# ictnlp/StreamSpeech

Measured on AMD Instinct MI355X. Metric: real-time factor (RTFx = audio seconds / wall seconds) + utterances/sec, offline S2ST fr-en, higher is better.
Workload: dtype f32

## Files before the change

streamspeech_amd/csrc/conv_c64w.hip:

```cpp
#include "slab_common.hpp"

#include <type_traits>

namespace ss {

using u32x4 = __attribute__((ext_vector_type(4))) unsigned;

#ifndef CW_TIMING
#define CW_TIMING 0
#endif
#if CW_TIMING
__device__ unsigned long long g_cw_dbg[1024 * 8];
#define CW_STAMP(k) do { if (t == 0) { const unsigned long long _n = __builtin_amdgcn_s_memtime(); cw_acc[k] += _n - cw_last; cw_last = _n; } } while (0)
#else
#define CW_STAMP(k) do { } while (0)
#endif

namespace {
constexpr int CW_MAXSEG = 256;
constexpr int CW_MAXROWS = 320;
constexpr int CW_MAXROWS_128 = 192;
[[maybe_unused]] constexpr int CW_NUM_RECORDS = 0x7ffffff0;
constexpr int cw_bme(int dil, int rows = 256) { return rows == 128 ? (dil == 1 ? 128 : dil == 3 ? 126 : 120) : (dil == 1 ? 256 : dil == 3 ? 252 : 240); }
[[maybe_unused]] __host__ __device__ constexpr int cw_nc(int kind) { return kind == 0 ? 4 : kind == 1 ? 2 : 3; }
[[maybe_unused]] __host__ __device__ constexpr int cw_slot(int kind, int n) { return kind == 0 ? n : kind == 1 ? (n == 0 ? 0 : 3) : (n == 2 ? 3 : n); }
[[maybe_unused]] __host__ __device__ constexpr int cw_ja(int kind, int n) { return kind == 0 ? (n == 3 ? 1 : n) : kind == 1 ? n : (n == 0 ? 0 : 1); }
[[maybe_unused]] __host__ __device__ constexpr int cw_jb(int kind, int n) { return kind == 0 ? (n == 2 ? 1 : n == 3 ? 3 : 2) : kind == 1 ? n : (n == 2 ? 2 : 1); }
[[maybe_unused]] __host__ __device__ constexpr int cw_op(int kind, int n) { return kind == 0 ? (n == 1 ? 1 : -1) : kind == 1 ? 0 : (n == 1 ? 0 : -1); }
}

__global__ void wino_pack_kernel(const float* __restrict__ W, float* __restrict__ WW, int C, int taps, int groups) {
  const int n = C * groups * C;
  for (int idx = blockIdx.x * blockDim.x + threadIdx.x; idx < n; idx += gridDim.x * blockDim.x) {
    const int ci = idx % C, g = (idx / C) % groups, co = idx / (C * groups);
    const float* w = W + (size_t)co * taps * C + ci;
    const float w0 = 3 * g < taps ? w[(size_t)(3 * g) * C] : 0.f;
    const float w1 = 3 * g + 1 < taps ? w[(size_t)(3 * g + 1) * C] : 0.f;
    const float w2 = 3 * g + 2 < taps ? w[(size_t)(3 * g + 2) * C] : 0.f;
    float* o = WW + (size_t)co * groups * 4 * C + (size_t)g * 4 * C + ci;
    const int left = taps - 3 * g;
    if (left >= 3) {
      o[0] = w0;
      o[C] = 0.5f * ((w0 + w1) + w2);
      o[2 * C] = 0.5f * ((w0 - w1) + w2);
      o[3 * C] = w2;
    } else if (left == 2) {
      o[0] = w0; o[C] = w0 + w1; o[2 * C] = 0.f; o[3 * C] = w1;
    } else {
      o[0] = w0; o[C] = 0.f; o[2 * C] = 0.f; o[3 * C] = -w0;
    }
  }
}

template <int DIL, int CH, int TAIL, int ROWS = 256>
__global__ __launch_bounds__(CH >= 128 ? 512 : 256, CH >= 128 ? 1 : CH == 64 ? 2 : 3) void conv_c64w_kernel(const GemmArgs p, const int groups, const int slab_rows) {
#if __HIP_DEVICE_COMPILE__
  constexpr int CS = CH == 256 ? 128 : CH;
  constexpr int KH = CH / CS;
  constexpr int C = CH, LDA = CS + 4, CT = CH >= 64 ? 4 : CH / 16, CB = CS / 16, RING = 2 * CT, TPR = CS / 4;
  constexpr int NT = CH >= 128 ? 512 : 256, RPP = NT / TPR;
  static_assert(ROWS == 256 || (ROWS == 128 && CH == 256), "half-height blocks: the 256-channel form only");
// ... 332 lines not shown
```

streamspeech_amd/csrc/debug_ops.hip:

```cpp
#include "model_internal.hpp"
#include "ctc_align.hpp"
#include "ctc_beam.hpp"

static int op_bind_wino(GemmArgs& a, void* stream) {
  static thread_local std::map<hipStream_t, DevBuf> wino_tmps;
  DevBuf& wino_tmp = wino_tmps[(hipStream_t)stream];
  const int N = a.N, Cin = a.Cin, taps = a.taps;
  if ((conv_c64w_enabled() && N == 64 && Cin == 64 && taps >= 3 && conv_c64_eligible(a)) ||
      (conv_c128w_enabled() && N == 128 && Cin == 128 && taps >= 3 && a.same_rows && !a.glu) ||
      (conv_c256w_enabled() && N == 256 && Cin == 256 && taps >= 3 && a.same_rows && !a.glu) ||
      (conv_c32w_enabled() && N == 32 && Cin == 32 && taps >= 3 && conv_c32_eligible(a))) {
    RET(wino_tmp.ensure((size_t)N * ((taps + 2) / 3) * 4 * N * sizeof(float)));
    RET(launch_wino_pack(a.W, wino_tmp.f(), N, taps, (hipStream_t)stream));
    a.Wwino = wino_tmp.f();
  }
  return SS_OK;
}

extern "C" int ss_op_conv_gemm(void* stream, const float* dA, int lda, const float* dW, const float* dbias,
                               const float* dR, int ldr, const float* dR2, int ldr2, float* dC, int ldc, int M,
                               int N, int Cin, int taps, int dil, int stride, int pad, int in_len, int chunk,
                               int in_act, float in_slope, int act, float alpha, float div, int glu) {
  GemmArgs a;
  a.A = dA; a.lda = lda; a.W = dW; a.bias = dbias; a.R = dR; a.ldr = ldr; a.R2 = dR2; a.ldr2 = ldr2; a.C = dC; a.ldc = ldc;
  a.M = M; a.N = N; a.Cin = Cin; a.taps = taps; a.dil = dil; a.stride = stride; a.pad = pad; a.in_len = in_len;
  a.chunk = chunk; a.in_act = in_act; a.in_slope = in_slope; a.act = act; a.alpha = alpha; a.div = div; a.glu = glu;
  a.same_rows = (stride == 1 && M == in_len) ? 1 : 0;
  RET(op_bind_wino(a, stream));
  return launch_conv_gemm(a, (hipStream_t)stream);
}

static void op_fill_conv(GemmArgs& a, const ss_op_conv_args* x) {
  a.A = x->A; a.W = x->W; a.bias = x->bias; a.R = x->R; a.R2 = x->R2; a.C = x->C; a.C2 = x->C2;
  a.lda = x->lda; a.ldc = x->ldc; a.ldr = x->ldr; a.ldr2 = x->ldr2; a.ldc2 = x->ldc2;
  a.M = x->M; a.N = x->N; a.Cin = x->Cin; a.taps = x->taps; a.dil = x->dil; a.stride = x->stride; a.pad = x->pad;
  a.in_len = x->in_len; a.chunk = x->chunk;
  a.in_act = x->in_act; a.in_slope = x->in_slope; a.act = x->act; a.act_slope = x->act_slope; a.alpha = x->alpha; a.div = x->div;
  a.c2_slope = x->c2_slope; a.glu = x->glu;
  a.segs = x->segs; a.nseg = x->nseg; a.max_seg_out = x->max_seg_out; a.same_rows = x->same_rows;
}
extern "C" int ss_op_conv_gemm_ex(void* stream, const ss_op_conv_args* x) {
  if (!x) return SS_ERR_ARG;
  GemmArgs a;
  op_fill_conv(a, x);
// ... 71 lines not shown
}
extern "C" int ss_op_ln_linear(void* stream, const float* dX, int ldx, const float* ln_g, const float* ln_b, const float* dW,
                               const float* dbias, const float* dR, int ldr, float* dC, int ldc, int M, int N, int K, int act,
                               float alpha, int glu) {
  GemmArgs a;
  a.A = dX; a.lda = ldx; a.W = dW; a.bias = dbias; a.R = dR; a.ldr = ldr; a.C = dC; a.ldc = ldc;
  a.M = M; a.N = N; a.Cin = K; a.in_len = M; a.act = act; a.alpha = alpha; a.glu = glu; a.same_rows = 1;
  a.ln_g = ln_g; a.ln_b = ln_b;
  return launch_conv_gemm(a, (hipStream_t)stream);
}
extern "C" int ss_op_ln_linear_ex(void* stream, const float* dX, int ldx, const float* ln_g, const float* ln_b, float* ln_out,
                                  const float* dW, const float* dbias, const float* dR, int ldr, float* dC, int ldc, int M, int N, int K,
                                  int act, float alpha, int glu, int canon) {
  if (canon < 0 || canon > 2 || (ln_g == nullptr) != (ln_b == nullptr) || (ln_out && !ln_g)) return SS_ERR_ARG;
  GemmArgs a;
  a.A = dX; a.lda = ldx; a.W = dW; a.bias = dbias; a.R = dR; a.ldr = ldr; a.C = dC; a.ldc = ldc;
  a.M = M; a.N = N; a.Cin = K; a.in_len = M; a.act = act; a.alpha = alpha; a.glu = glu; a.same_rows = 1;
  a.ln_g = ln_g; a.ln_b = ln_b; a.ln_out = ln_out; a.canon = canon;
  return launch_conv_gemm(a, (hipStream_t)stream);
}
extern "C" int ss_debug_conv_c64(int enable) {
  if (enable == 4 || enable == 5) { conv_c64w_debug(enable == 5); return SS_OK; }
  if (enable == 6 || enable == 7) { conv_c128w_debug(enable == 7); return SS_OK; }
  if (enable == 8 || enable == 9) { conv_c256w_debug(enable == 9); return SS_OK; }
  conv_c64_debug(enable);
  return SS_OK;
}
extern "C" int ss_debug_conv_c256_rows(int rows) { return conv_c256w_rows_debug(rows); }
extern "C" int ss_debug_conv_c32(int enable) {
  if (enable == 4 || enable == 5) { conv_c32w_debug(enable == 5); return SS_OK; }
  conv_c32_debug(enable);
  return SS_OK;
}
extern "C" int ss_debug_conv_c16(int enable) { conv_c16_debug(enable); return SS_OK; }
extern "C" int64_t ss_debug_enc_step_launches(void) { return (int64_t)enc_step_launch_count(); }
extern "C" int ss_debug_scratch_audit(ss_scratch* sc, size_t* booked, size_t* held) {
  if (!sc || !booked || !held) return SS_ERR_ARG;
  size_t sum = 0;
  bool foreign = false;
  for (DevBuf* b : sc->all()) {
    sum += b->bytes;
    if (b->acct != &sc->acct) foreign = true;
  }
  *booked = sc->acct.used;
  *held = sum;
  return foreign ? SS_ERR_ARG : SS_OK;
}
extern "C" int ss_debug_rtlin(int grid, int enable) {
  if (grid < 0) return SS_ERR_ARG;
  rtlin_debug(grid, enable);
  return SS_OK;
}
extern "C" int ss_debug_rtlin_kb(int uw, int order) {
  if (!(uw == 0 || uw == 1 || uw == 2 || uw == 4) || order < -1 || order > 2) return SS_ERR_ARG;
  rtlin_kb_debug(uw, order);
  return SS_OK;
}
extern "C" int ss_debug_rtlin_kb_last(int32_t out[4]) {
  if (!out) return SS_ERR_ARG;
  int v[4];
  rtlin_kb_last(v);
  for (int i = 0; i < 4; ++i) out[i] = v[i];
  return SS_OK;
}
extern "C" int ss_debug_unit_l0_distinct(int on) {
  if (on < -1 || on > 1) return SS_ERR_ARG;
  dispatch_edit([on](Dispatch& d) { d.unit_l0_distinct = on < 0 ? (getenv("SS_UNIT_L0_DISTINCT") ? atoi(getenv("SS_UNIT_L0_DISTINCT")) != 0 : 1) : on; });
// ... 218 lines not shown
```

streamspeech_amd/csrc/dispatch.hip:

```cpp
#include "gemm.hpp"

#include <atomic>
#include <cstdlib>
#include <map>
#include <mutex>
#include <utility>
#include <vector>

namespace ss {

namespace {
std::mutex g_disp_mu;
std::atomic<unsigned> g_disp_gen{1};
Dispatch env_defaults() {
  Dispatch d;
  auto I = [](const char* k, int dflt) { const char* e = getenv(k); return e ? atoi(e) : dflt; };
  auto L = [](const char* k, long long dflt) { const char* e = getenv(k); return e ? atoll(e) : dflt; };
  d.attn_split = I("SS_ATTN_NO_SPLIT", 0) ? -1 : 0; d.attn_q16 = I("SS_ATTN_Q16", d.attn_q16);
  d.c16_off = I("SS_NO_CONV_C16", 0) ? 1 : 0; d.c32_off = I("SS_NO_CONV_C32", 0) ? 1 : 0; d.c64_off = I("SS_NO_CONV_C64", 0) ? 1 : 0;
  d.c16_min_rows = L("SS_CONV_C16_MIN_ROWS", d.c16_min_rows); d.c32_min_rows = L("SS_CONV_C32_MIN_ROWS", d.c32_min_rows);
  d.c64_min_rows = L("SS_CONV_C64_MIN_ROWS", d.c64_min_rows);
  d.c64w_on = I("SS_CONV_C64_WINOGRAD", 1); d.c128w_on = I("SS_CONV_C128_WINOGRAD", 1); d.c256w_on = I("SS_CONV_C256_WINOGRAD", 1);
  d.c32w_on = I("SS_CONV_C32_WINOGRAD", 1); d.c64w_min_k = I("SS_CONV_C64_WINOGRAD_MIN_K", 3);
  d.c128w_min_rows = L("SS_CONV_C128_MIN_ROWS", d.c128w_min_rows); d.c256w_min_rows = L("SS_CONV_C256_MIN_ROWS", d.c256w_min_rows);
  if (const int r = I("SS_CONV_C256_ROWS", d.c256w_rows); r == 128 || r == 256) d.c256w_rows = r;
  if (getenv("SS_FFN_WM")) { d.ffn_wm = I("SS_FFN_WM", 3); d.ffn_wm_forced = 1; d.ffn_wm_env = d.ffn_wm; }
  d.ffn_fusion = I("SS_NO_FFN_FUSION", 0) ? 0 : 1; d.ffn_min_rows = I("SS_FFN_MIN_ROWS", d.ffn_min_rows);
  if (getenv("SS_SK_MIN_GFLOP")) d.sk_min_flops = 1e9 * atof(getenv("SS_SK_MIN_GFLOP"));
  d.no_resblock_fusion = I("SS_NO_RESBLOCK_FUSION", 0); d.no_pair_fusion = I("SS_NO_PAIR_FUSION", 0);
  d.rt_off = I("SS_NO_RTLIN", 0) ? 1 : 0; d.rt_min_rows = I("SS_RTLIN_MIN_ROWS", d.rt_min_rows); d.rt_min_units = L("SS_RTLIN_MIN_UNITS", d.rt_min_units);
  d.rt_kb_min_units = L("SS_RTLIN_KB_MIN_UNITS", d.rt_kb_min_units); d.rt_kb_uw = I("SS_RTLIN_KB_UW", d.rt_kb_uw); d.rt_kb_xmap = I("SS_RTLIN_KB_XMAP", d.rt_kb_xmap);
  d.smallm_max_rows = I("SS_SMALLM_MAX_ROWS", d.smallm_max_rows); d.sk_min_units = L("SS_SK_MIN_UNITS", d.sk_min_units);
  d.no_sk2 = I("SS_NO_SK2", 0) ? 1 : 0; d.sk2_min_k64 = I("SS_SK2_MINK64", d.sk2_min_k64); d.sk2_spare_cus = I("SS_SK2_SPARE_CUS", 0);
  d.rt_wg_per_cu = I("SS_RTLIN_WG_PER_CU", 0); d.c32_min_k = I("SS_CONV_C32_MIN_K", d.c32_min_k); d.c16_min_k = I("SS_CONV_C16_MIN_K", d.c16_min_k);
  d.unit_l0_distinct = I("SS_UNIT_L0_DISTINCT", 1) ? 1 : 0; d.fbank_dense = I("SS_FBANK_DENSE", 0) ? 1 : 0;
  return d;
}
Dispatch& process_settings() { static Dispatch d = env_defaults(); return d; }
thread_local const Dispatch* t_disp = nullptr;
thread_local CtxDispatch t_disp_own;
}
void dispatch_edit(const std::function<void(Dispatch&)>& fn) {
  std::lock_guard<std::mutex> lk(g_disp_mu);
  fn(process_settings());
  g_disp_gen.fetch_add(1, std::memory_order_release);
}
void slab_debug(int grid, long long min_rows) {
  const Dispatch dflt = env_defaults();
  dispatch_edit([=](Dispatch& d) {
    d.slab_grid_cap = grid > 0 ? grid : 0;
    const bool set = min_rows >= 0;
    d.c16_min_rows = set ? min_rows : dflt.c16_min_rows; d.c32_min_rows = set ? min_rows : dflt.c32_min_rows;
    d.c64_min_rows = set ? min_rows : dflt.c64_min_rows;
    d.c128w_min_rows = set ? min_rows : dflt.c128w_min_rows; d.c256w_min_rows = set ? min_rows : dflt.c256w_min_rows;
  });
}
// ... 120 lines not shown
```

streamspeech_amd/csrc/dispatch.hpp:

```cpp
#pragma once
#include <functional>

namespace ss {

struct Dispatch {
  int attn_no_mfma = 0;
  int attn_q16 = 1;
  int attn_split = 0;
  int c16_off = 0, c32_off = 0, c64_off = 0;
  long long c16_min_rows = 131072, c32_min_rows = 65536, c64_min_rows = 32768;
  int c64w_on = 1, c128w_on = 1, c256w_on = 1, c32w_on = 1;
  int c64w_min_k = 3;
  long long c128w_min_rows = 65536, c256w_min_rows = 32768;
  int c256w_rows = 128;
  int c32_min_k = 7, c16_min_k = 11;
  int slab_grid_cap = 0;
  int sk_groups = 0;
  int sk2_spare_cus = 0;
  int ffn_force_g = 0;
  int ffn_wm = 3, ffn_wm_forced = 0;
  int ffn_wm_env = 0;
  int ffn_fusion = 1;
  int ffn_min_rows = 1000;
  int force_bm = 0, force_bn = 0, force_ks = 0;
  double sk_min_flops = 4e9;
  int smallm_max_rows = 192;
  long long sk_min_units = 12 * 512;
  int no_sk2 = 0;
  int sk2_min_k64 = 192;
  int no_resblock_fusion = 0, no_pair_fusion = 0;
  int rt_off = 0, rt_min_rows = 193, rt_force_g = 0;
  long long rt_min_units = 4000;
  int rt_wg_per_cu = 0;
  long long rt_kb_min_units = 256;
  int rt_kb_xmap = 1;
  int rt_kb_uw = 0;
  int rt_kb_order = 1;
  int unit_l0_distinct = 1;
  int fbank_dense = 0;
};

const Dispatch& disp();
void dispatch_edit(const std::function<void(Dispatch&)>& fn);

struct CtxDispatch {
// ... 12 lines not shown
```

streamspeech_amd/csrc/gemm.hip:

```cpp
#include "gemm.hpp"

#include <type_traits>

namespace ss {

using f32x4 = __attribute__((ext_vector_type(4))) float;

template <int BM, int BN, int BK, int WM, int WN, int KS, int PD, bool BLK = false>
__global__ __launch_bounds__(256 * KS) void conv_gemm_kernel(const GemmArgs p) {
  static_assert(WM * WN == 4, "4 waves per k-group");
  static_assert(!BLK || KS == 1, "the blocked chain is the KS = 1 form");
  constexpr int LDK = BK + 8;
  constexpr int WTM = BM / WM, WTN = BN / WN;
  constexpr int TM = WTM / 16, TN = WTN / 16;
  static_assert(TM >= 1 && TN >= 1, "wave tile must hold a 16x16 MFMA tile");
  constexpr int KQ = BK / 4;
  constexpr int A_F4 = BM * KQ, W_F4 = BN * KQ;
  constexpr int NA = (A_F4 + 255) / 256, NW = (W_F4 + 255) / 256;
  constexpr int STAGE = (BM + BN) * LDK;
  extern __shared__ __attribute__((aligned(16))) float smem_all[];
  const int kg = threadIdx.x >> 8;
  float* smem = smem_all + kg * 2 * STAGE;

  const int t = threadIdx.x & 255, lane = t & 63, wave = t >> 6;
// ... 660 lines not shown
  return plain_linear(a) && M <= disp().smallm_max_rows && M > 0;
}


int launch_conv_gemm(const GemmArgs& a_in, hipStream_t stream) {
  GemmArgs a = a_in;
  const int M = a.nseg > 0 ? a.max_seg_out : a.M;
  if (M <= 0 || a.N <= 0) return SS_OK;
  if (a.Wf16) return launch_conv_f16(a, stream);
  if (a.Cin % 16 != 0 || (a.lda & 3) != 0 || a.taps < 1) return SS_ERR_ARG;
  if (a.glu && (a.N % 32 != 0 || a.C2)) return SS_ERR_ARG;
  const bool k32 = (a.Cin % 32) == 0;
  const int nseg = a.nseg > 0 ? a.nseg : 1;
  if (a.canon == CANON_NONE) a.canon = canon_mode();
  if (a.canon != CANON_NONE && !disp().force_bm) { a.m_begin = 0; return launch_canon(a, stream); }
  if (a.seg_mb || a.seg_A) return SS_ERR_ARG;
  if (a.m_begin > 0) {
    if (a.nseg > 0 || a.m_begin >= a.M || a.ln_g || a.ln_out || a.N <= 32) return SS_ERR_ARG;
    return launch_32x64<false>(a, stream, (long)cdiv(a.M - a.m_begin, 32) * cdiv(a.N, 64));
  }
  if ((!disp().force_bm || a.ln_out) && gemv_eligible(a)) return launch_gemv(a, stream);
  if (a.ln_out) return SS_ERR_ARG;
  if (smallm_eligible(a)) {
    if (a.glu) return launch_smallm<2, 2, true>(a, stream, PROF_SMALLM_2x2);
    const long wgs16 = (long)cdiv(M, 16) * cdiv(a.N, 16);
    if (a.Cin >= 1024 || wgs16 <= 1024) return launch_smallm<4, 1>(a, stream, PROF_SMALLM_4x1);
    if (wgs16 <= 4096) return launch_smallm<2, 2>(a, stream, PROF_SMALLM_2x2);
    return launch_smallm<1, 4>(a, stream, PROF_SMALLM_1x4);
  }
  if (!disp().force_bm && conv_c64_eligible(a)) return conv_c64w_eligible(a) ? launch_conv_c64w(a, stream) : launch_conv_c64(a, stream);
  if (!disp().force_bm && conv_wide_winograd_eligible(a, 128)) return launch_conv_c128w(a, stream);
  if (!disp().force_bm && conv_wide_winograd_eligible(a, 256)) return launch_conv_c256w(a, stream);
  if (!disp().force_bm && conv_c32_eligible(a)) return conv_c32w_eligible(a) ? launch_conv_c32w(a, stream) : launch_conv_c32(a, stream);
  if (!disp().force_bm && conv_c16_eligible(a)) return launch_conv_c16(a, stream);
  if (!disp().force_bm && rtlin_eligible(a)) return launch_rtlin(a, stream);
  if (a.ln_g) return SS_ERR_ARG;
  if (disp().force_bm == 1 && conv_sk_eligible(a)) return launch_conv_sk(a, stream, disp().force_ks);
  if (disp().force_bm == 4 && conv_sk2_eligible(a)) return launch_conv_sk2(a, stream, disp().force_ks);
  if (disp().force_bm == 5 && conv_sk2_eligible(a)) { GemmArgs b = a; b.x3 = 1; return launch_conv_sk2(b, stream, disp().force_ks); }
  if (!disp().force_bm && conv_sk_eligible(a) && 2.0 * (double)a.M * a.N * a.taps * a.Cin >= disp().sk_min_flops) {
    const long long nk = (long long)a.taps * (a.Cin / 32);
    const bool wide = a.N % 128 == 0;
    const long long units = (long long)cdiv(a.M, 128) * (a.N / (wide ? 128 : 64)) * nk;
    const long long min_units = disp().sk_min_units;
    if (!disp().no_sk2 && conv_sk2_eligible(a) && (wide ? units >= min_units : a.taps * a.Cin >= disp().sk2_min_k64)) return launch_conv_sk2(a, stream);
    if (wide ? units >= min_units : a.taps * a.Cin >= 448) return launch_conv_sk(a, stream);
  }
  if (disp().force_bm && a.N > 32 && k32) {
    const int f = disp().force_bm * 10000 + (disp().force_bn % 100) * 100 + disp().force_ks;
    switch (f) {
#define SS_CASE(BM_, BN_, KS_, PD_, CLS_) case BM_ * 10000 + BN_ * 100 + KS_ * 10 + PD_: return launch_cfg<BM_, BN_, 32, 2, 2, KS_, PD_>(a, stream, CLS_);
      SS_CASE(64, 64, 1, 1, PROF_GEMM_64x64x32) SS_CASE(64, 64, 1, 2, PROF_GEMM_64x64x32) SS_CASE(64, 64, 1, 3, PROF_GEMM_64x64x32)
      SS_CASE(64, 64, 2, 2, PROF_GEMM_64x64x32) SS_CASE(64, 64, 2, 3, PROF_GEMM_64x64x32)
      SS_CASE(32, 64, 1, 1, PROF_GEMM_32x64x32) SS_CASE(32, 64, 1, 2, PROF_GEMM_32x64x32) SS_CASE(32, 64, 1, 3, PROF_GEMM_32x64x32) SS_CASE(32, 64, 1, 4, PROF_GEMM_32x64x32)
      SS_CASE(32, 64, 2, 3, PROF_GEMM_32x64x32) SS_CASE(32, 64, 4, 3, PROF_GEMM_32x64x32)
      SS_CASE(32, 32, 1, 1, PROF_GEMM_32x32x32) SS_CASE(32, 32, 1, 2, PROF_GEMM_32x32x32) SS_CASE(32, 32, 1, 3, PROF_GEMM_32x32x32) SS_CASE(32, 32, 1, 4, PROF_GEMM_32x32x32)
      SS_CASE(32, 32, 2, 3, PROF_GEMM_32x32x32) SS_CASE(32, 32, 4, 3, PROF_GEMM_32x32x32)
#undef SS_CASE
      case 128 * 10000 + 28 * 100 + 11: return launch_cfg<128, 128, 16, 2, 2, 1, 1>(a, stream, PROF_GEMM_128x128x16);
      case 128 * 10000 + 64 * 100 + 11: return launch_cfg<128, 64, 32, 2, 2, 1, 1>(a, stream, PROF_GEMM_128x64x32);
      default: break;
    }
  }
  if (disp().force_bm != 2 && conv_slab_eligible(a) && a.M >= 2048) return launch_conv_slab(a, stream);
  return launch_tiles<false>(a, stream, M, nseg);
}

// ... 2 lines not shown
```

streamspeech_amd/csrc/gemm.hpp:

```cpp
#pragma once
#include "common.hpp"
#include "dispatch.hpp"
#include "prof.hpp"

namespace ss {

struct GemmArgs {
  const float* A = nullptr;
  const float* W = nullptr;
  const float* Wwino = nullptr;
  const void* Wf16 = nullptr;
  const float* bias = nullptr;
  const float* R = nullptr;
  const float* R2 = nullptr;
  float* C = nullptr;
  int lda = 0, ldc = 0, ldr = 0, ldr2 = 0;
  int M = 0, N = 0, Cin = 0;
  int taps = 1, dil = 1, stride = 1, pad = 0;
  int in_len = 0;
  int chunk = 0;
  int m_begin = 0;
  int in_act = ACT_NONE;
  float in_slope = 0.1f;
  int act = ACT_NONE;
// ... 89 lines not shown
                          int taps, int M, float slope, const int* segs, int nseg, hipStream_t stream);

bool conv_c64_eligible(const GemmArgs& a);
bool conv_c64_enabled();
int launch_conv_c64(const GemmArgs& a, hipStream_t stream);
bool conv_c64w_eligible(const GemmArgs& a);
int launch_conv_c64w(const GemmArgs& a, hipStream_t stream);
int launch_wino_pack(const float* W, float* WW, int C, int taps, hipStream_t stream);
void conv_c64w_debug(int enable);
bool conv_c64w_enabled();
bool conv_wide_winograd_eligible(const GemmArgs& a, int ch);
int launch_conv_c128w(const GemmArgs& a, hipStream_t stream);
void conv_c128w_debug(int enable);
bool conv_c128w_enabled();
int launch_conv_c256w(const GemmArgs& a, hipStream_t stream);
void conv_c256w_debug(int enable);
int conv_c256w_rows_debug(int rows);
bool conv_c256w_enabled();
bool conv_c32w_eligible(const GemmArgs& a);
int launch_conv_c32w(const GemmArgs& a, hipStream_t stream);
void conv_c32w_debug(int enable);
bool conv_c32w_enabled();
void conv_c64_debug(int enable);

bool conv_c32_eligible(const GemmArgs& a);
bool conv_c32_enabled();
int launch_conv_c32(const GemmArgs& a, hipStream_t stream);
void conv_c32_debug(int enable);

bool conv_c16_eligible(const GemmArgs& a);
bool conv_c16_enabled();
int launch_conv_c16(const GemmArgs& a, hipStream_t stream);
void conv_c16_debug(int enable);

bool conv_f16_eligible(const GemmArgs& a);
bool conv_f16_geometry_ok(int C, int taps, int dil);
int launch_conv_f16(const GemmArgs& a, hipStream_t stream);
size_t f16_pack_halves(int C, int taps);
int launch_f16_pack(const float* W, void* Wf, int C, int taps, hipStream_t stream);

bool rtlin_eligible(const GemmArgs& a);
bool rtlin_shape_ok(const GemmArgs& a);
int launch_rtlin(const GemmArgs& a, hipStream_t stream);
void rtlin_debug(int grid, int enable);
bool rtlin_kb_shape_ok(const GemmArgs& a);
bool rtlin_kb_eligible(const GemmArgs& a);
int launch_rtlin_kb(const GemmArgs& a, hipStream_t stream);
void rtlin_kb_debug(int uw, int order);
void rtlin_kb_last(int out[4]);

bool ffn_fused_eligible(int D, int F, int act, int M, int ldx, int ldy, bool canon = false);
int launch_ffn_fused(const float* X, int ldx, float* Y, int ldy, const float* ln_g, const float* ln_b, const float* W1,
                     const float* b1, const float* W2, const float* b2, float alpha, const float* ln2_g, const float* ln2_b,
                     int M, int D, int F, hipStream_t stream, int canon = 0);
void ffn_fused_debug_grid(int g);
void ffn_fused_debug_rows(int wm);

bool gemv_eligible(const GemmArgs& a);
bool smallm_eligible(const GemmArgs& a);

void debug_force_tile(int bm, int bn, int ks);
bool debug_tile_forced();

int launch_conv_gemm(const GemmArgs& a, hipStream_t stream);

}
// ... 1 lines not shown
```

streamspeech_amd/csrc/prof.hip:

```cpp
#include "gemm.hpp"

#include <atomic>
#include <cstdio>
#include <cstdlib>
#include <cstring>
#include <map>
#include <mutex>
#include <string>
#include <tuple>
#include <utility>
#include <vector>

namespace ss {

static const char* kTileNames[] = {
    "conv_gemm<128,16,16,4,1>", "conv_gemm<128,32,32,4,1>", "conv_gemm<128,32,16,4,1>", "conv_gemm<16,128,32,1,4>",
    "conv_gemm<16,128,16,1,4>", "conv_gemm<128,128,16,2,2>", "conv_gemm<128,64,32,2,2>", "conv_gemm<64,64,32,2,2>",
    "conv_gemm<64,64,16,2,2>", "conv_gemm<32,64,32,2,2>", "conv_gemm<32,64,16,2,2>", "conv_gemm<32,32,32,2,2>",
    "smallm_gemm<4,1>", "smallm_gemm<2,2>", "smallm_gemm<1,4>", "conv_sk<128,BN,32>",
    "conv_slab<32>", "conv_slab<16>", "conv_sk2<256,128,32>", "conv_sk2_bf16x3<256,128,32>",
    "resblock_fused<32>", "resblock_fused<16>", "ffn_fused<256,2048>", "rt_linear<48,256>", "conv_c64<256,64>", "conv_c32<256,32>", "conv_c16<256,16>", "conv_c64w<256,64>", "conv_c128w<256,128>", "conv_c32w<256,32>", "conv_c256w<256,128>", "rt_linear_kb<48,256>",
    "conv_f16<64>", "conv_f16<128>", "conv_f16<256>"};
static_assert(sizeof(kTileNames) / sizeof(kTileNames[0]) == kNumTileCfg, "one name per ProfCls, in enum order");
static std::atomic<int> g_prof_mask{0};
static std::atomic<int> g_prof_mask_hi{0};
static std::vector<ProfRec> g_prof_recs;
static std::vector<std::pair<hipEvent_t, hipEvent_t>> g_prof_pool;
static std::mutex g_prof_mu;

void prof_enable(int cls_mask) { g_prof_mask.store(cls_mask, std::memory_order_relaxed); }
void prof_enable_hi(int cls_mask) { g_prof_mask_hi.store(cls_mask, std::memory_order_relaxed); }
const char* prof_cfg_name(int cls) { return (cls >= 0 && cls < kNumTileCfg) ? kTileNames[cls] : "?"; }
void prof_reset() {
  for (auto& r : g_prof_recs) g_prof_pool.push_back({r.e0, r.e1});
  g_prof_recs.clear();
}
int prof_read_issued(int cls, double* issued) {
  double v = 0;
  for (auto& r : g_prof_recs) if (r.cls == cls) v += r.issued;
  if (issued) *issued = v;
  return SS_OK;
}
int prof_read(int cls, double* ms_total, double* flops_total, long long* launches, double* bytes_total) {
  double ms = 0, fl = 0, by = 0; long long n = 0;
  for (auto& r : g_prof_recs) {
    if (r.cls != cls) continue;
    if (hipEventSynchronize(r.e1) != hipSuccess) return SS_ERR_HIP;
    float t = 0.f;
    if (hipEventElapsedTime(&t, r.e0, r.e1) != hipSuccess) return SS_ERR_HIP;
    ms += t; fl += r.flops; by += r.bytes; ++n;
  }
  if (ms_total) *ms_total = ms;
  if (flops_total) *flops_total = fl;
  if (launches) *launches = n;
  if (bytes_total) *bytes_total = by;
// ... 23 lines not shown
  FILE* f = path ? fopen(path, "w") : nullptr;
  if (!f) return;
  std::lock_guard<std::mutex> lk(g_tot_mu);
  fputs(shape_table().c_str(), f);
  fclose(f);
}
static std::atomic<int> g_shape_log{getenv("SS_SHAPE_LOG") != nullptr ? 1 : 0};
void prof_shape_log(int on) {
  std::lock_guard<std::mutex> lk(g_tot_mu);
  if (on && g_shapes && !getenv("SS_SHAPE_LOG")) g_shapes->clear();
  g_shape_log.store(on ? 1 : 0, std::memory_order_relaxed);
}
int prof_shape_dump(char* buf, int cap) {
  std::lock_guard<std::mutex> lk(g_tot_mu);
  const std::string t = shape_table();
  if (buf && cap > 0) { const int n = (int)std::min<size_t>(t.size(), (size_t)cap - 1); memcpy(buf, t.data(), n); buf[n] = 0; }
  return (int)t.size() + 1;
}
int prof_totals(int cls, double* flops, double* bytes, long long* launches) {
  if (cls < 0 || cls >= kNumTileCfg) return SS_ERR_ARG;
  if (flops) *flops = (double)g_prof_totals[cls].flops.load(std::memory_order_relaxed);
  if (bytes) *bytes = (double)g_prof_totals[cls].bytes.load(std::memory_order_relaxed);
  if (launches) *launches = (long long)g_prof_totals[cls].launches.load(std::memory_order_relaxed);
  return SS_OK;
}
static void algo_work(const GemmArgs& a, double& flops, double& bytes) {
  flops = a.algo_flops > 0 ? a.algo_flops : 2.0 * (double)a.M * a.N * a.taps * a.Cin;
  const double ncols = a.glu ? a.N / 2 : a.N;
  bytes = 4.0 * ((double)a.N * a.taps * a.Cin + (a.bias ? a.N : 0) + (double)a.in_len * a.Cin +
                 (double)a.M * ncols * (1 + (a.R ? 1 : 0) + (a.R2 ? 1 : 0)));
  if (a.algo_bytes > 0) bytes = a.algo_bytes;
}

static bool prof_cls_winograd(ProfCls cls) { return cls >= PROF_CONV_C64W && cls <= PROF_CONV_C256W; }

int prof_begin(const GemmArgs& a, hipStream_t stream, ProfCls cls, ProfRec& rec, bool& prof) {
  {
    double fl, by;
    algo_work(a, fl, by);
    g_prof_totals[cls].flops.fetch_add((unsigned long long)(fl + 0.5), std::memory_order_relaxed);
    g_prof_totals[cls].bytes.fetch_add((unsigned long long)(by + 0.5), std::memory_order_relaxed);
    g_prof_totals[cls].launches.fetch_add(1ull, std::memory_order_relaxed);
    if (g_shape_log.load(std::memory_order_relaxed)) {
      std::lock_guard<std::mutex> lk(g_tot_mu);
      if (!g_shapes) { g_shapes = new std::map<ShapeKey, ShapeTot>(); if (getenv("SS_SHAPE_LOG")) atexit(shape_log_dump); }
      const int ops = (a.R ? 1 : 0) | (a.R2 ? 2 : 0) | (a.C2 ? 4 : 0) | (a.in_act != ACT_NONE ? 8 : 0) | (a.act != ACT_NONE ? 16 : 0) | (a.glu ? 32 : 0) | (a.nseg > 0 ? 64 : 0);
      ShapeTot& z = (*g_shapes)[ShapeKey(cls, a.N, a.taps, a.Cin, ops)];
      z.launches += 1; z.rows += a.M; z.flops += fl; z.bytes += by;
    }
  }
  prof = cls < 32 ? ((unsigned)g_prof_mask.load(std::memory_order_relaxed) >> cls) & 1u
                  : ((unsigned)g_prof_mask_hi.load(std::memory_order_relaxed) >> (cls - 32)) & 1u;
  if (!prof) return SS_OK;
  std::lock_guard<std::mutex> lk(g_prof_mu);
  if (!g_prof_pool.empty()) { rec.e0 = g_prof_pool.back().first; rec.e1 = g_prof_pool.back().second; g_prof_pool.pop_back(); }
  else { SS_HIP_CHECK(hipEventCreate(&rec.e0)); SS_HIP_CHECK(hipEventCreate(&rec.e1)); }
  rec.cls = cls;
  algo_work(a, rec.flops, rec.bytes);
  rec.issued = (prof_cls_winograd(cls) && a.taps >= 3) ? rec.flops * (4.0 * (a.taps / 3) + (a.taps % 3 ? a.taps % 3 + 1 : 0)) / (2.0 * a.taps) : rec.flops;
  SS_HIP_CHECK(hipEventRecord(rec.e0, stream));
  return SS_OK;
}
int prof_end(hipStream_t stream, ProfRec& rec, bool prof) {
  if (prof) {
    std::lock_guard<std::mutex> lk(g_prof_mu);
    SS_HIP_CHECK(hipEventRecord(rec.e1, stream));
    g_prof_recs.push_back(rec);
// ... 6 lines not shown
```

streamspeech_amd/csrc/prof.hpp:

```cpp
#pragma once
#include "common.hpp"

namespace ss {

struct GemmArgs;

enum ProfCls : int {
  PROF_GEMM_128x16x16 = 0, PROF_GEMM_128x32x32 = 1, PROF_GEMM_128x32x16 = 2, PROF_GEMM_16x128x32 = 3, PROF_GEMM_16x128x16 = 4,
  PROF_GEMM_128x128x16 = 5, PROF_GEMM_128x64x32 = 6, PROF_GEMM_64x64x32 = 7, PROF_GEMM_64x64x16 = 8, PROF_GEMM_32x64x32 = 9,
  PROF_GEMM_32x64x16 = 10, PROF_GEMM_32x32x32 = 11,
  PROF_SMALLM_4x1 = 12, PROF_SMALLM_2x2 = 13, PROF_SMALLM_1x4 = 14,
  PROF_CONV_SK = 15, PROF_CONV_SLAB32 = 16, PROF_CONV_SLAB16 = 17, PROF_CONV_SK2 = 18, PROF_CONV_SK2_BF16X3 = 19,
  PROF_RESBLOCK32 = 20, PROF_RESBLOCK16 = 21, PROF_FFN = 22, PROF_RTLIN = 23,
  PROF_CONV_C64 = 24, PROF_CONV_C32 = 25, PROF_CONV_C16 = 26,
  PROF_CONV_C64W = 27, PROF_CONV_C128W = 28, PROF_CONV_C32W = 29, PROF_CONV_C256W = 30,
  PROF_RTLIN_KB = 31,
  PROF_CONV_F16_64 = 32, PROF_CONV_F16_128 = 33, PROF_CONV_F16_256 = 34,
};
constexpr int kNumTileCfg = PROF_CONV_F16_256 + 1;
void prof_enable(int cls_mask);
void prof_enable_hi(int cls_mask);
void prof_reset();
int prof_read(int cls, double* ms_total, double* flops_total, long long* launches, double* bytes_total = nullptr);
const char* prof_cfg_name(int cls);
int prof_totals(int cls, double* flops, double* bytes, long long* launches);
int prof_read_issued(int cls, double* issued_flops_total);
void prof_shape_log(int on);
int prof_shape_dump(char* buf, int cap);

struct ProfRec { hipEvent_t e0, e1; double flops, bytes, issued; int cls; };
int prof_begin(const GemmArgs& a, hipStream_t stream, ProfCls cls, ProfRec& rec, bool& prof);
int prof_end(hipStream_t stream, ProfRec& rec, bool prof);

}
```

streamspeech_amd/csrc/vocoder.hip:

```cpp
#include "model_internal.hpp"

#include <cstdint>
#include <tuple>


namespace {
struct WinoShared { DevBuf buf; size_t floats = 0; int refs = 0; };
struct WinoKey {
  int dev; const float* blob; uint64_t sig;
  bool operator<(const WinoKey& o) const { return std::tie(dev, blob, sig) < std::tie(o.dev, o.blob, o.sig); }
};
std::mutex g_wino_mu;
std::map<WinoKey, WinoShared> g_wino;
inline uint64_t fnv(uint64_t h, uint64_t v) { for (int i = 0; i < 8; ++i) { h ^= (v >> (8 * i)) & 0xff; h *= 1099511628211ull; } return h; }
uint64_t blob_sig(const ss_vocoder* v, const float* d_blob) {
  const ss_vocoder_config* cfg = &v->cfg;
  uint64_t sig = fnv(fnv(fnv(14695981039346656037ull, (uint64_t)cfg->upsample_initial_channel), (uint64_t)cfg->n_up), (uint64_t)cfg->n_res);
  for (int j = 0; j < cfg->n_res; ++j) sig = fnv(sig, (uint64_t)cfg->resblock_kernel_sizes[j]);
  for (size_t i = 0; i < v->rb_c1.size(); ++i) sig = fnv(fnv(sig, (uint64_t)(v->rb_c1[i].w - d_blob)), (uint64_t)(v->rb_c2[i].w - d_blob));
  return sig;
}
std::mutex g_f16_mu;
std::map<WinoKey, WinoShared> g_f16;
bool f16_stage(int ch) { return ch == 64 || ch == 128 || ch == 256; }
// ... 18 lines not shown
  v->dur_ln2 = {w.get("voc.dur.ln2.g", Hd), w.get("voc.dur.ln2.b", Hd)};
  v->dur_proj = {w.get("voc.dur.proj.w", Hd), w.get("voc.dur.proj.b", 1)};
  const int C0 = cfg->upsample_initial_channel;
  v->pre = {w.get("voc.pre.w", (int64_t)C0 * 7 * cfg->model_in_dim), w.get("voc.pre.b", C0)};
  int C = C0;
  for (int i = 0; i < cfg->n_up; ++i) {
    const int Co = C / 2, st = cfg->upsample_rates[i];
    v->ups.push_back({w.get("voc.up" + std::to_string(i) + ".w", (int64_t)st * Co * 3 * C),
                      w.get("voc.up" + std::to_string(i) + ".b", (int64_t)st * Co)});
    for (int j = 0; j < cfg->n_res; ++j) {
      const int kr = cfg->resblock_kernel_sizes[j];
      for (int dd = 0; dd < 3; ++dd) {
        const std::string p = "voc.rb" + std::to_string(i * cfg->n_res + j);
        v->rb_c1.push_back({w.get(p + ".c1." + std::to_string(dd) + ".w", (int64_t)Co * kr * Co),
                            w.get(p + ".c1." + std::to_string(dd) + ".b", Co)});
        v->rb_c2.push_back({w.get(p + ".c2." + std::to_string(dd) + ".w", (int64_t)Co * kr * Co),
                            w.get(p + ".c2." + std::to_string(dd) + ".b", Co)});
      }
    }
    C = Co;
  }
  v->post = {w.get("voc.post.w", (int64_t)7 * C), w.get("voc.post.b", 1)};
  {
    auto it = w.map.find("voc.spkr.table");
    if (it != w.map.end()) {
      const int64_t per = (int64_t)16 * C0;
      if (it->second.n <= 0 || it->second.n % per || it->second.n / per > INT32_MAX || (C0 & 3)) { scratch_unref(v->sc); delete v; return SS_ERR_ARG; }
      v->spk_table = it->second.p;
      v->n_spk = (int)(it->second.n / per);
    }
  }
  if (!w.missing.empty()) { scratch_unref(v->sc); delete v; return SS_ERR_MISSING_WEIGHT; }
  {
    auto wino_stage = [](int ch) { return ch == 32 || ch == 64 || ch == 128 || ch == 256; };
    size_t need = 0;
    int Cs = C0;
    for (int i = 0; i < cfg->n_up; ++i) {
      Cs /= 2;
      if (wino_stage(Cs)) for (int j = 0; j < cfg->n_res; ++j) need += 6 * (size_t)Cs * ((cfg->resblock_kernel_sizes[j] + 2) / 3) * 4 * Cs;
    }
    if (need) {
      int dev = 0;
      if (hipGetDevice(&dev) != hipSuccess) { scratch_unref(v->sc); delete v; return SS_ERR_HIP; }
      std::lock_guard<std::mutex> lk(g_wino_mu);
      const WinoKey key{dev, d_blob, blob_sig(v, d_blob)};
      WinoShared& sh = g_wino[key];
      const bool fresh = sh.refs == 0;
      if (!fresh && sh.floats != need) { scratch_unref(v->sc); delete v; return SS_ERR_ARG; }
      if (fresh) {
        rc = sh.buf.ensure(need * sizeof(float));
        if (rc != SS_OK) { g_wino.erase(key); scratch_unref(v->sc); delete v; return rc; }
        sh.floats = need;
      }
      float* dst = sh.buf.f();
      Cs = C0;
      for (int i = 0; i < cfg->n_up && rc == SS_OK; ++i) {
        Cs /= 2;
        if (!wino_stage(Cs)) continue;
        for (int j = 0; j < cfg->n_res && rc == SS_OK; ++j) {
          const int kr = cfg->resblock_kernel_sizes[j];
          const size_t n = (size_t)Cs * ((kr + 2) / 3) * 4 * Cs;
          for (int dd = 0; dd < 3 && rc == SS_OK; ++dd) {
            const int idx = (i * cfg->n_res + j) * 3 + dd;
            if (fresh) rc = launch_wino_pack(v->rb_c1[idx].w, dst, Cs, kr, nullptr);
            v->rb_c1[idx].ww = dst; dst += n;
            if (fresh && rc == SS_OK) rc = launch_wino_pack(v->rb_c2[idx].w, dst, Cs, kr, nullptr);
            v->rb_c2[idx].ww = dst; dst += n;
// ... 683 lines not shown
```

Baseline: 6497.

## Add Winograd F(2,3) kernel for 16-channel vocoder convolutions

Adds a 16-channel Winograd conv kernel (conv_c16w) that uses MFMA 16x16x4 f32 over prepacked Winograd weights and routes eligible c16 convolutions to it. The vocoder now precomputes Winograd-packed weights for 16-channel stages too. The aim is fewer multiplies in the last upsample stage's resblock convolutions than the direct slab kernel needs. Shared Winograd helper constants move into a common header. The trade-off is extra weight-packing memory and a new code path with different numerics.

```diff
diff --git a/streamspeech_amd/csrc/conv_c16w.hip b/streamspeech_amd/csrc/conv_c16w.hip
--- /dev/null
+++ b/streamspeech_amd/csrc/conv_c16w.hip
@@ -0,0 +1,219 @@
+#include "slab_common.hpp"
+#include "wino_kinds.hpp"
+
+#include <cstdlib>
+#include <type_traits>
+
+namespace ss {
+
+namespace {
+constexpr int C1W_C = 16;
+constexpr int C1W_LDA = C1W_C + 4;
+constexpr int C1W_MAXSEG = 256;
+constexpr int C1W_MAXROWS = 320;
+[[maybe_unused]] constexpr int C1W_NP =C1W_MAXROWS * (C1W_C / 4) / 256;
+
+template <int I, int N, class F>
+__device__ __forceinline__ void c1w_static_for(F&& f) {
+  if constexpr (I < N) {
+    f(std::integral_constant<int, I>{});
+    c1w_static_for<I + 1, N>(f);
+  }
+}
+}
+
+template <int DIL, int TAPS>
+__global__ __launch_bounds__(256, 3) void conv_c16w_kernel(const GemmArgs p, const int slab_rows) {
+#if __HIP_DEVICE_COMPILE__
+  constexpr int C = C1W_C, LDA = C1W_LDA, NP = C1W_NP;
+  constexpr int BME = cw_bme(DIL), NPAIR = BME / 2;
+  constexpr int NGF = TAPS / 3, TAIL = TAPS % 3, GROUPS = NGF + (TAIL ? 1 : 0);
+  constexpr int NFRAG = 4 * NGF + (TAIL ? cw_nc(TAIL) : 0), Kw = GROUPS * 4 * C;
+  static_assert(NGF >= 1, "the first group is a full one");
+  extern __shared__ __attribute__((aligned(16))) float smem[];
+  float* sA = smem;
+  int* s_blk = reinterpret_cast<int*>(smem + ((slab_rows * LDA + 3) & ~3));
+
+  const int t = threadIdx.x, lane = t & 63;
+  const int wave = __builtin_amdgcn_readfirstlane(t >> 6);
+  const int r = lane & 15, g = lane >> 4;
+
+  SlabWalk<GemmArgs> w(p, s_blk, BME);
+  __syncthreads();
+  const int nblocks = w.nblocks();
+  const float slope = p.in_act == ACT_LRELU ? p.in_slope : 1.0f;
+
+  int blk = blockIdx.x;
+  if (blk >= nblocks) return;
+  f32x4 wf[NFRAG];
+  c1w_static_for<0, GROUPS>([&](auto G) {
+    constexpr int GI = decltype(G)::value, K = GI < NGF ? 0 : TAIL;
+#pragma unroll
+    for (int n = 0; n < cw_nc(K); ++n)
+      wf[4 * GI + n] = *reinterpret_cast<const f32x4*>(p.W + (size_t)r * Kw + (GI * 4 + cw_slot(K, n)) * C + 4 * g);
+  });
+
+  int toff[2];
+  bool pv[2];
+#pragma unroll
+  for (int i = 0; i < 2; ++i) {
+    const int pp = wave * 32 + i * 16 + r;
+    pv[i] = pp < NPAIR;
+    const int pc = pv[i] ? pp : NPAIR - 1;
+    toff[i] = 2 * DIL * (pc / DIL) + pc % DIL;
+  }
+
+  for (; blk < nblocks; blk += gridDim.x) {
+    w.locate(blk, p.in_len);
+    const int m0 = w.m0, seg_lo = w.seg_lo, seg_hi = w.seg_hi;
+    const int m_hi = p.nseg > 0 ? seg_hi : min(seg_hi, p.M);
+    const bool edge = (m0 - p.pad < seg_lo) || (m0 - p.pad + slab_rows > seg_hi);
+    __syncthreads();
+    {
+      f32x4 pre[NP];
+#pragma unroll
+      for (int u = 0; u < NP; ++u) {
+        const int rho = (t >> 2) + 64 * u;
+        const int gc = min(max(m0 - p.pad + rho, seg_lo), seg_hi - 1);
+        pre[u] = *reinterpret_cast<const f32x4*>(p.A + (size_t)gc * p.lda + (t & 3) * 4);
+      }
+      float* dst = sA + (t >> 2) * LDA + (t & 3) * 4;
+#pragma unroll
+      for (int u = 0; u < NP; ++u) {
+        const int rho = (t >> 2) + 64 * u;
+        f32x4 v = pre[u];
+        if (edge) {
+          const int gin = m0 - p.pad + rho;
+          const bool ok = gin >= seg_lo && gin < seg_hi;
+#pragma unroll
+          for (int e = 0; e < 4; ++e) v[e] = ok ? v[e] : 0.f;
+        }
+#pragma unroll
+        for (int e = 0; e < 4; ++e) v[e] = fmaxf(v[e], v[e] * slope);
+        if (rho < slab_rows) *reinterpret_cast<f32x4*>(dst + u * 64 * LDA) = v;
+      }
+    }
+    __syncthreads();
+
+    f32x4 acc[2][4];
+#pragma unroll
+    for (int i = 0; i < 2; ++i)
+#pragma unroll
+      for (int f = 0; f < 4; ++f) acc[i][f] = f32x4{0.f, 0.f, 0.f, 0.f};
+    auto xform = [&](int op, const f32x4 a, const f32x4 b) -> f32x4 { return op == 1 ? a + b : op == 0 ? a : a - b; };
+    auto group = [&](auto KIND, auto G, const f32x4 (&x)[4], f32x4 (&m)[4]) __attribute__((always_inline)) {
+      constexpr int K = decltype(KIND)::value, NC = cw_nc(K), F0 = 4 * decltype(G)::value;
+      f32x4 xa[NC];
+#pragma unroll
+      for (int n = 0; n < NC; ++n) xa[n] = xform(cw_op(K, n), x[cw_ja(K, n)], x[cw_jb(K, n)]);
+#pragma unroll
+      for (int e = 0; e < 4; ++e)
+#pragma unroll
+        for (int n = 0; n < NC; ++n)
+          m[cw_slot(K, n)] = __builtin_amdgcn_mfma_f32_16x16x4f32(wf[F0 + n][e], xa[n][e], m[cw_slot(K, n)], 0, 0, 0);
+    };
+#pragma unroll
+    for (int i = 0; i < 2; ++i) {
+      const float* pa = sA + toff[i] * LDA + 4 * g;
+      auto rd = [&](int j) -> f32x4 { return *reinterpret_cast<const f32x4*>(pa + j * DIL * LDA); };
+      f32x4 x[4];
+      x[0] = rd(0);
+      c1w_static_for<0, NGF>([&](auto G) {
+        constexpr int GI = decltype(G)::value;
+        x[1] = rd(3 * GI + 1); x[2] = rd(3 * GI + 2); x[3] = rd(3 * GI + 3);
+        group(std::integral_constant<int, 0>{}, G, x, acc[i]);
+        x[0] = x[3];
+      });
+      if constexpr (TAIL == 1) {
+        x[1] = rd(3 * NGF + 1);
+        group(std::integral_constant<int, 1>{}, std::integral_constant<int, NGF>{}, x, acc[i]);
+      }
+      if constexpr (TAIL == 2) {
+        x[1] = rd(3 * NGF + 1); x[2] = rd(3 * NGF + 2);
+        group(std::integral_constant<int, 2>{}, std::integral_constant<int, NGF>{}, x, acc[i]);
+      }
+    }
+
+    int le = lane;
+    asm volatile("" : "+v"(le));
+    const int cole = (le >> 4) * 4;
+    f32x4 y[4];
+    int mrow[4];
+#pragma unroll
+    for (int i = 0; i < 2; ++i) {
+      y[i * 2] = (acc[i][0] + acc[i][1]) + acc[i][2];
+      y[i * 2 + 1] = (acc[i][1] - acc[i][2]) - acc[i][3];
+      mrow[i * 2] = m0 + toff[i];
+      mrow[i * 2 + 1] = m0 + toff[i] + DIL;
+    }
+    f32x4 bb[1] = {f32x4{0.f, 0.f, 0.f, 0.f}};
+    if (p.bias) bb[0] = *reinterpret_cast<const f32x4*>(p.bias + cole);
+    slab_epi_batch(p, y, bb, [&](int q, int n) -> size_t {
+      return (size_t)min(mrow[n], m_hi - 1) * (q == 0 ? p.ldr : p.ldr2) + cole;
+    });
+#pragma unroll
+    for (int q = 0; q < 4; ++q) {
+      if (pv[q / 2] && mrow[q] < m_hi) slab_epi_store<false>(p, mrow[q], cole, y[q]);
+    }
+  }
+#endif
+}
+
+void conv_c16w_debug(int enable) {
+  dispatch_edit([enable](Dispatch& d) {
+    const Dispatch dflt;
+    const char* e = getenv("SS_CONV_C16_WINOGRAD");
+    const char* k = getenv("SS_CONV_C16_WINOGRAD_MIN_K");
+    d.c16w_on = enable < 0 ? (e ? atoi(e) : dflt.c16w_on) : enable ? 1 : 0;
+    d.c16w_op = enable == 2 ? 1 : 0;
+    d.c16w_min_k = enable == 2 ? 3 : (k ? atoi(k) : dflt.c16w_min_k);
+  });
+}
+bool conv_c16w_enabled() { return disp().c16w_on != 0; }
+bool conv_c16w_op_enabled() { return disp().c16w_on != 0 && disp().c16w_op != 0; }
+
+static int c1w_slab_rows(const GemmArgs& a) { return cw_bme(a.dil) + (a.taps - 1) * a.dil; }
+
+bool conv_c16w_eligible(const GemmArgs& a) {
+  const Dispatch& d = disp();
+  if (!d.c16w_on || !a.Wwino || a.taps < 3 || a.taps < (d.c16w_min_k > 0 ? d.c16w_min_k : d.c16_min_k)) return false;
+  if ((a.dil != 1 && a.dil != 3 && a.dil != 5) || a.C2 || a.pad != a.dil * (a.taps - 1) / 2) return false;
+  return c1w_slab_rows(a) <= C1W_MAXROWS && 3 * slab_lds_bytes(c1w_slab_rows(a), C1W_LDA, C1W_MAXSEG) <= 158 * 1024;
+}
+
+template <int DIL, int TAPS>
+static int launch_c16w_t(GemmArgs a, hipStream_t stream) {
+  constexpr int BME = cw_bme(DIL);
+  const int slab_rows = BME + (TAPS - 1) * DIL;
+  const size_t lds = slab_lds_bytes(slab_rows, C1W_LDA, C1W_MAXSEG);
+  SkWorkspace* st = nullptr;
+  int rc = sk_workspace_acquire(stream, &st);
+  if (rc != SS_OK) return rc;
+  const int grid = slab_grid(3, st->cus, a.M, BME, a.nseg);
+  ProfRec rec{}; bool prof = false;
+  rc = prof_begin(a, stream, PROF_CONV_C16W, rec, prof);
+  if (rc != SS_OK) return rc;
+  a.W = a.Wwino;
+  hipLaunchKernelGGL((conv_c16w_kernel<DIL, TAPS>), dim3(grid), dim3(256), lds, stream, a, slab_rows);
+  SS_LAUNCH_CHECK();
+  return prof_end(stream, rec, prof);
+}
+
+int launch_conv_c16w(const GemmArgs& a, hipStream_t stream) {
+  if (!conv_c16_eligible(a) || !conv_c16w_eligible(a)) return SS_ERR_ARG;
+  if (a.in_act != ACT_NONE && a.in_act != ACT_LRELU) return SS_ERR_ARG;
+  switch (a.dil * 100 + a.taps) {
+    case 103: return launch_c16w_t<1, 3>(a, stream);
+    case 107: return launch_c16w_t<1, 7>(a, stream);
+    case 111: return launch_c16w_t<1, 11>(a, stream);
+    case 303: return launch_c16w_t<3, 3>(a, stream);
+    case 307: return launch_c16w_t<3, 7>(a, stream);
+    case 311: return launch_c16w_t<3, 11>(a, stream);
+    case 503: return launch_c16w_t<5, 3>(a, stream);
+    case 507: return launch_c16w_t<5, 7>(a, stream);
+    case 511: return launch_c16w_t<5, 11>(a, stream);
+    default: return SS_ERR_ARG;
+  }
+}
+
+}
diff --git a/streamspeech_amd/csrc/conv_c64w.hip b/streamspeech_amd/csrc/conv_c64w.hip
--- a/streamspeech_amd/csrc/conv_c64w.hip
+++ b/streamspeech_amd/csrc/conv_c64w.hip
@@ -1,4 +1,5 @@
 #include "slab_common.hpp"
+#include "wino_kinds.hpp"
 
 #include <type_traits>
 
@@ -21,12 +22,6 @@
 constexpr int CW_MAXROWS = 320;
 constexpr int CW_MAXROWS_128 = 192;
 [[maybe_unused]] constexpr int CW_NUM_RECORDS = 0x7ffffff0;
-constexpr int cw_bme(int dil, int rows = 256) { return rows == 128 ? (dil == 1 ? 128 : dil == 3 ? 126 : 120) : (dil == 1 ? 256 : dil == 3 ? 252 : 240); }
-[[maybe_unused]] __host__ __device__ constexpr int cw_nc(int kind) { return kind == 0 ? 4 : kind == 1 ? 2 : 3; }
-[[maybe_unused]] __host__ __device__ constexpr int cw_slot(int kind, int n) { return kind == 0 ? n : kind == 1 ? (n == 0 ? 0 : 3) : (n == 2 ? 3 : n); }
-[[maybe_unused]] __host__ __device__ constexpr int cw_ja(int kind, int n) { return kind == 0 ? (n == 3 ? 1 : n) : kind == 1 ? n : (n == 0 ? 0 : 1); }
-[[maybe_unused]] __host__ __device__ constexpr int cw_jb(int kind, int n) { return kind == 0 ? (n == 2 ? 1 : n == 3 ? 3 : 2) : kind == 1 ? n : (n == 2 ? 2 : 1); }
-[[maybe_unused]] __host__ __device__ constexpr int cw_op(int kind, int n) { return kind == 0 ? (n == 1 ? 1 : -1) : kind == 1 ? 0 : (n == 1 ? 0 : -1); }
 }
 
 __global__ void wino_pack_kernel(const float* __restrict__ W, float* __restrict__ WW, int C, int taps, int groups) {
diff --git a/streamspeech_amd/csrc/debug_ops.hip b/streamspeech_amd/csrc/debug_ops.hip
--- a/streamspeech_amd/csrc/debug_ops.hip
+++ b/streamspeech_amd/csrc/debug_ops.hip
@@ -9,7 +9,8 @@
   if ((conv_c64w_enabled() && N == 64 && Cin == 64 && taps >= 3 && conv_c64_eligible(a)) ||
       (conv_c128w_enabled() && N == 128 && Cin == 128 && taps >= 3 && a.same_rows && !a.glu) ||
       (conv_c256w_enabled() && N == 256 && Cin == 256 && taps >= 3 && a.same_rows && !a.glu) ||
-      (conv_c32w_enabled() && N == 32 && Cin == 32 && taps >= 3 && conv_c32_eligible(a))) {
+      (conv_c32w_enabled() && N == 32 && Cin == 32 && taps >= 3 && conv_c32_eligible(a)) ||
+      (conv_c16w_op_enabled() && N == 16 && Cin == 16 && taps >= 3 && conv_c16_eligible(a))) {
     RET(wino_tmp.ensure((size_t)N * ((taps + 2) / 3) * 4 * N * sizeof(float)));
     RET(launch_wino_pack(a.W, wino_tmp.f(), N, taps, (hipStream_t)stream));
     a.Wwino = wino_tmp.f();
@@ -147,7 +148,11 @@
   conv_c32_debug(enable);
   return SS_OK;
 }
-extern "C" int ss_debug_conv_c16(int enable) { conv_c16_debug(enable); return SS_OK; }
+extern "C" int ss_debug_conv_c16(int enable) {
+  if (enable >= 4 && enable <= 6) { conv_c16w_debug(enable == 4 ? 0 : enable == 5 ? 2 : -1); return SS_OK; }
+  conv_c16_debug(enable);
+  return SS_OK;
+}
 extern "C" int64_t ss_debug_enc_step_launches(void) { return (int64_t)enc_step_launch_count(); }
 extern "C" int ss_debug_scratch_audit(ss_scratch* sc, size_t* booked, size_t* held) {
   if (!sc || !booked || !held) return SS_ERR_ARG;
diff --git a/streamspeech_amd/csrc/dispatch.hip b/streamspeech_amd/csrc/dispatch.hip
--- a/streamspeech_amd/csrc/dispatch.hip
+++ b/streamspeech_amd/csrc/dispatch.hip
@@ -22,6 +22,7 @@
   d.c64_min_rows = L("SS_CONV_C64_MIN_ROWS", d.c64_min_rows);
   d.c64w_on = I("SS_CONV_C64_WINOGRAD", 1); d.c128w_on = I("SS_CONV_C128_WINOGRAD", 1); d.c256w_on = I("SS_CONV_C256_WINOGRAD", 1);
   d.c32w_on = I("SS_CONV_C32_WINOGRAD", 1); d.c64w_min_k = I("SS_CONV_C64_WINOGRAD_MIN_K", 3);
+  d.c16w_on = I("SS_CONV_C16_WINOGRAD", d.c16w_on) ? 1 : 0; d.c16w_min_k = I("SS_CONV_C16_WINOGRAD_MIN_K", d.c16w_min_k);
   d.c128w_min_rows = L("SS_CONV_C128_MIN_ROWS", d.c128w_min_rows); d.c256w_min_rows = L("SS_CONV_C256_MIN_ROWS", d.c256w_min_rows);
   if (const int r = I("SS_CONV_C256_ROWS", d.c256w_rows); r == 128 || r == 256) d.c256w_rows = r;
   if (getenv("SS_FFN_WM")) { d.ffn_wm = I("SS_FFN_WM", 3); d.ffn_wm_forced = 1; d.ffn_wm_env = d.ffn_wm; }
diff --git a/streamspeech_amd/csrc/dispatch.hpp b/streamspeech_amd/csrc/dispatch.hpp
--- a/streamspeech_amd/csrc/dispatch.hpp
+++ b/streamspeech_amd/csrc/dispatch.hpp
@@ -11,6 +11,7 @@
   long long c16_min_rows = 131072, c32_min_rows = 65536, c64_min_rows = 32768;
   int c64w_on = 1, c128w_on = 1, c256w_on = 1, c32w_on = 1;
   int c64w_min_k = 3;
+  int c16w_on = 1, c16w_op = 0, c16w_min_k = 0;
   long long c128w_min_rows = 65536, c256w_min_rows = 32768;
   int c256w_rows = 128;
   int c32_min_k = 7, c16_min_k = 11;
diff --git a/streamspeech_amd/csrc/gemm.hip b/streamspeech_amd/csrc/gemm.hip
--- a/streamspeech_amd/csrc/gemm.hip
+++ b/streamspeech_amd/csrc/gemm.hip
@@ -716,7 +716,7 @@
   if (!disp().force_bm && conv_wide_winograd_eligible(a, 128)) return launch_conv_c128w(a, stream);
   if (!disp().force_bm && conv_wide_winograd_eligible(a, 256)) return launch_conv_c256w(a, stream);
   if (!disp().force_bm && conv_c32_eligible(a)) return conv_c32w_eligible(a) ? launch_conv_c32w(a, stream) : launch_conv_c32(a, stream);
-  if (!disp().force_bm && conv_c16_eligible(a)) return launch_conv_c16(a, stream);
+  if (!disp().force_bm && conv_c16_eligible(a)) return conv_c16w_eligible(a) ? launch_conv_c16w(a, stream) : launch_conv_c16(a, stream);
   if (!disp().force_bm && rtlin_eligible(a)) return launch_rtlin(a, stream);
   if (a.ln_g) return SS_ERR_ARG;
   if (disp().force_bm == 1 && conv_sk_eligible(a)) return launch_conv_sk(a, stream, disp().force_ks);
diff --git a/streamspeech_amd/csrc/gemm.hpp b/streamspeech_amd/csrc/gemm.hpp
--- a/streamspeech_amd/csrc/gemm.hpp
+++ b/streamspeech_amd/csrc/gemm.hpp
@@ -145,6 +145,11 @@
 bool conv_c16_enabled();
 int launch_conv_c16(const GemmArgs& a, hipStream_t stream);
 void conv_c16_debug(int enable);
+bool conv_c16w_eligible(const GemmArgs& a);
+int launch_conv_c16w(const GemmArgs& a, hipStream_t stream);
+void conv_c16w_debug(int enable);
+bool conv_c16w_enabled();
+bool conv_c16w_op_enabled();
 
 bool conv_f16_eligible(const GemmArgs& a);
 bool conv_f16_geometry_ok(int C, int taps, int dil);
diff --git a/streamspeech_amd/csrc/prof.hip b/streamspeech_amd/csrc/prof.hip
--- a/streamspeech_amd/csrc/prof.hip
+++ b/streamspeech_amd/csrc/prof.hip
@@ -20,7 +20,7 @@
     "smallm_gemm<4,1>", "smallm_gemm<2,2>", "smallm_gemm<1,4>", "conv_sk<128,BN,32>",
     "conv_slab<32>", "conv_slab<16>", "conv_sk2<256,128,32>", "conv_sk2_bf16x3<256,128,32>",
     "resblock_fused<32>", "resblock_fused<16>", "ffn_fused<256,2048>", "rt_linear<48,256>", "conv_c64<256,64>", "conv_c32<256,32>", "conv_c16<256,16>", "conv_c64w<256,64>", "conv_c128w<256,128>", "conv_c32w<256,32>", "conv_c256w<256,128>", "rt_linear_kb<48,256>",
-    "conv_f16<64>", "conv_f16<128>", "conv_f16<256>"};
+    "conv_f16<64>", "conv_f16<128>", "conv_f16<256>", "conv_c16w<256,16>"};
 static_assert(sizeof(kTileNames) / sizeof(kTileNames[0]) == kNumTileCfg, "one name per ProfCls, in enum order");
 static std::atomic<int> g_prof_mask{0};
 static std::atomic<int> g_prof_mask_hi{0};
@@ -110,7 +110,7 @@
   if (a.algo_bytes > 0) bytes = a.algo_bytes;
 }
 
-static bool prof_cls_winograd(ProfCls cls) { return cls >= PROF_CONV_C64W && cls <= PROF_CONV_C256W; }
+static bool prof_cls_winograd(ProfCls cls) { return (cls >= PROF_CONV_C64W && cls <= PROF_CONV_C256W) || cls == PROF_CONV_C16W; }
 
 int prof_begin(const GemmArgs& a, hipStream_t stream, ProfCls cls, ProfRec& rec, bool& prof) {
   {
diff --git a/streamspeech_amd/csrc/prof.hpp b/streamspeech_amd/csrc/prof.hpp
--- a/streamspeech_amd/csrc/prof.hpp
+++ b/streamspeech_amd/csrc/prof.hpp
@@ -16,8 +16,9 @@
   PROF_CONV_C64W = 27, PROF_CONV_C128W = 28, PROF_CONV_C32W = 29, PROF_CONV_C256W = 30,
   PROF_RTLIN_KB = 31,
   PROF_CONV_F16_64 = 32, PROF_CONV_F16_128 = 33, PROF_CONV_F16_256 = 34,
+  PROF_CONV_C16W = 35,
 };
-constexpr int kNumTileCfg = PROF_CONV_F16_256 + 1;
+constexpr int kNumTileCfg = PROF_CONV_C16W + 1;
 void prof_enable(int cls_mask);
 void prof_enable_hi(int cls_mask);
 void prof_reset();
diff --git a/streamspeech_amd/csrc/vocoder.hip b/streamspeech_amd/csrc/vocoder.hip
--- a/streamspeech_amd/csrc/vocoder.hip
+++ b/streamspeech_amd/csrc/vocoder.hip
@@ -74,7 +74,7 @@
   }
   if (!w.missing.empty()) { scratch_unref(v->sc); delete v; return SS_ERR_MISSING_WEIGHT; }
   {
-    auto wino_stage = [](int ch) { return ch == 32 || ch == 64 || ch == 128 || ch == 256; };
+    auto wino_stage = [](int ch) { return ch == 16 || ch == 32 || ch == 64 || ch == 128 || ch == 256; };
     size_t need = 0;
     int Cs = C0;
     for (int i = 0; i < cfg->n_up; ++i) {
diff --git a/streamspeech_amd/csrc/wino_kinds.hpp b/streamspeech_amd/csrc/wino_kinds.hpp
--- /dev/null
+++ b/streamspeech_amd/csrc/wino_kinds.hpp
@@ -0,0 +1,12 @@
+#pragma once
+
+namespace ss {
+
+constexpr int cw_bme(int dil, int rows = 256) { return rows == 128 ? (dil == 1 ? 128 : dil == 3 ? 126 : 120) : (dil == 1 ? 256 : dil == 3 ? 252 : 240); }
+__host__ __device__ constexpr int cw_nc(int kind) { return kind == 0 ? 4 : kind == 1 ? 2 : 3; }
+__host__ __device__ constexpr int cw_slot(int kind, int n) { return kind == 0 ? n : kind == 1 ? (n == 0 ? 0 : 3) : (n == 2 ? 3 : n); }
+__host__ __device__ constexpr int cw_ja(int kind, int n) { return kind == 0 ? (n == 3 ? 1 : n) : kind == 1 ? n : (n == 0 ? 0 : 1); }
+__host__ __device__ constexpr int cw_jb(int kind, int n) { return kind == 0 ? (n == 2 ? 1 : n == 3 ? 3 : 2) : kind == 1 ? n : (n == 2 ? 2 : 1); }
+__host__ __device__ constexpr int cw_op(int kind, int n) { return kind == 0 ? (n == 1 ? 1 : -1) : kind == 1 ? 0 : (n == 1 ? 0 : -1); }
+
+}
```

Result: no change. 6519 (median of 2 runs) (+0.3%).
